# chanchanchan97/ICAFusion

Measured on NVIDIA H100. Metric: 640x512 RGB+IR pairs/sec end-to-end, higher is better.
Workload: dtype f16

## Files before the change

### icafusion_b200/_lib.py

```python
from __future__ import annotations

import ctypes as C
import os

_HERE = os.path.dirname(os.path.abspath(__file__))
LIB_PATH = os.path.join(_HERE, "libicaf_b200.so")

ACT_NONE, ACT_SILU, ACT_GELU = 0, 1, 2
EPI_BIAS_ROW, EPI_ADD_RES, EPI_SCALED_RES, EPI_LN_FOLD, EPI_EMIT_STATS = 1, 2, 4, 8, 16


class ConvGeom(C.Structure):
    _fields_ = [(n, C.c_int) for n in ("B", "Hi", "Wi", "Cin", "Ho", "Wo", "Cout", "kh", "kw", "stride", "pad",
                                       "k_pad", "w_rows", "act", "epi")]


class ConvIO(C.Structure):
    _fields_ = [("x", C.c_void_p), ("x_ld", C.c_int64), ("w", C.c_void_p), ("bias", C.c_void_p),
                ("res", C.c_void_p), ("res_ld", C.c_int64), ("y", C.c_void_p), ("y_ld", C.c_int64),
                ("alpha", C.c_void_p), ("beta", C.c_void_p),
                ("ln_stats", C.c_void_p), ("ln_colsum", C.c_void_p), ("ln_parts", C.c_int), ("ln_eps", C.c_float),
                ("stats_out", C.c_void_p)]


class ConvPlan(C.Structure):
    _fields_ = [(n, C.c_int) for n in ("kernel", "bn", "a_mode", "tile_w", "tile_h", "tiles_x", "tiles_y", "cblk", "halo",
                                       "stages", "splits", "grid_x", "grid_y", "grid_z", "cluster", "smem_bytes",
                                       "work_items", "ctas")]


class BottleneckIO(C.Structure):
    _fields_ = [("x", C.c_void_p), ("x_ld", C.c_int64), ("w1", C.c_void_p), ("b1", C.c_void_p), ("w3", C.c_void_p),
                ("b2", C.c_void_p), ("y", C.c_void_p), ("y_ld", C.c_int64)]


class LossHyp(C.Structure):
    _fields_ = [(n, C.c_float) for n in ("box", "obj", "cls", "cls_pw", "obj_pw", "anchor_t", "fl_gamma", "gr", "cp", "cn")] + \
               [("balance", C.c_float * 5)]


class AugTile(C.Structure):
    _fields_ = [("rgb", C.c_void_p), ("ir", C.c_void_p)] + \
               [(n, C.c_int) for n in ("H0", "W0", "h", "w", "x1a", "y1a", "x2a", "y2a", "x1b", "y1b", "xtab", "ytab")]


class AugSample(C.Structure):
    _fields_ = [("tile", AugTile * 4)] + [(n, C.c_int) for n in ("ntiles", "canvas", "warp", "flipud", "fliplr", "reserved")] + \
               [("lut", C.c_uint8 * (2 * 3 * 256))]


class ValSample(C.Structure):
    _fields_ = [("rgb", C.c_void_p), ("ir", C.c_void_p)] + \
               [(n, C.c_int) for n in ("H0", "W0", "h", "w", "top", "left", "mode", "xtab", "ytab", "sx", "sy", "reserved")]


KERNEL_TC = 0

_vp, _i, _i64, _f = C.c_void_p, C.c_int, C.c_int64, C.c_float
SIGNATURES = {
    "icaf_version": [],
    "icaf_last_error": [],
    "icaf_sm_count": [],
    "icaf_kernel_launches": [],
    "icaf_conv2d_fwd": [C.POINTER(ConvGeom), C.POINTER(ConvIO), _i, _vp],
    "icaf_conv2d_plan": [C.POINTER(ConvGeom), _i, _i, _i, C.POINTER(ConvPlan)],
    "icaf_conv2d_fwd_simt": [C.POINTER(ConvGeom), C.POINTER(ConvIO), _i, _vp],
    "icaf_bottleneck_fwd": [_i, _i, _i, C.POINTER(BottleneckIO), _i, _vp],
    "icaf_pack_image": [_vp, _i, _f, _i, _i, _i, _vp, _vp],
    "icaf_pack_image_s2d": [_vp, _i, _f, _i, _i, _i, _vp, _vp],
    "icaf_letterbox": [_vp, _i, _i, _i, _vp, _i, _i, _i, _i, _i, _i, _vp, _vp, _i, _vp],
    "icaf_sppf_pool": [_vp, _i64, _vp, _vp, _vp, _i64, _i, _i, _i, _i, _vp],
    "icaf_upsample2x": [_vp, _i64, _vp, _i64, _i, _i, _i, _i, _vp],
    "icaf_copy_channels": [_vp, _i64, _vp, _i64, _i64, _i, _vp],
    "icaf_prefetch_l2": [_vp, C.c_size_t, _vp],
    "icaf_dmff_pool_tokens": [_vp, _vp, _i64, _vp, _vp, _vp, _vp, _vp, _vp, _vp, _i, _i, _i, _i, _i, _i, _i, _vp],
    "icaf_row_stats": [_vp, _vp, _vp, _vp, _i64, _i, _vp],
    "icaf_layernorm": [_vp, _vp, _vp, _vp, _vp, _vp, _vp, _vp, _i64, _i, _f, _vp],
    "icaf_cross_attention": [_vp, _vp, _vp, _vp, _vp, _vp, _i, _i, _i, _i, _i, _vp],
    "icaf_cross_attention_simt": [_vp, _vp, _vp, _vp, _vp, _vp, _i, _i, _i, _i, _i, _vp],
    "icaf_dmff_upsample_cat": [_vp, _vp, _i, _vp, _vp, _i64, _vp, _i64, _i, _i, _i, _i, _i, _i, _i, _vp],
    "icaf_nms_workspace_bytes": [_i, _i],
    "icaf_nms": [_vp, _i, _i, _i, _f, _f, _i, C.c_uint64, _i, _vp, _vp, _vp, C.c_size_t, _vp],
    "icaf_nms_multi_label_workspace_bytes": [_i, _i, _i],
    "icaf_nms_multi_label": [_vp, _i, _i, _i, _f, _f, _i, C.c_uint64, _i, _vp, _vp, _vp, C.c_size_t, _vp],
    "icaf_match_detections_workspace_bytes": [_i],
    "icaf_match_detections": [_vp, _vp, _i, _i, _vp, _i, _vp, _i, _i, _vp, _i, _i, _vp, _vp, _vp, C.c_size_t, _vp],
    "icaf_kaist_mr_workspace_bytes": [_i, _i, _i],
    "icaf_kaist_mr": [_vp, _vp, _vp, _vp, _vp, _vp, _i, _i, _i, _vp, _vp, _i, _i, _vp, _vp, _vp, _vp, C.c_size_t, _vp],
    "icaf_kaist_round_detections": [_vp, _vp, _vp, _vp, _i, _i, _i, _vp, _vp, _vp],
    "icaf_loss_workspace_bytes": [_i, _i, _i, C.POINTER(C.c_int), C.POINTER(C.c_int), _i, _i],
    "icaf_compute_loss_fwd": [C.POINTER(C.c_void_p), _i, _i, C.POINTER(C.c_int), C.POINTER(C.c_int), _i, _i, _i, _i, _vp, _i,
                              C.POINTER(C.c_float), C.POINTER(LossHyp), _vp, _vp, C.c_size_t, _vp],
    "icaf_compute_loss_bwd": [C.POINTER(C.c_void_p), _i, _i, C.POINTER(C.c_int), C.POINTER(C.c_int), _i, _i, _i, _i, _vp, _i,
                              C.POINTER(C.c_float), C.POINTER(LossHyp), _vp, C.POINTER(C.c_void_p), _vp, C.c_size_t, _vp],
    "icaf_conv2d_wgrad_workspace_bytes": [C.POINTER(ConvGeom)],
    "icaf_conv2d_wgrad": [C.POINTER(ConvGeom), _vp, _i64, _vp, _i64, _vp, _f, _i, _vp, C.c_size_t, _vp],
    "icaf_zero_stuff2": [_vp, _vp, _i, _i, _i, _i, _i, _i, _vp],
    "icaf_colsum": [_vp, _i64, _i, _vp, _f, _i, _vp, C.c_size_t, _vp],
    "icaf_train_workspace_bytes": [_i],
    "icaf_bn_act_fwd": [_vp, _vp, _vp, _vp, _vp, _vp, _vp, _vp, _i64, _i, _f, _f, _i, _vp, C.c_size_t, _vp],
    "icaf_bn_act_bwd": [_vp, _vp, _vp, _vp, _vp, _vp, _vp, _vp, _vp, _i64, _i, _i, _f, _i, _vp, C.c_size_t, _vp],
    "icaf_bn_act_fwd_stats": [_vp, _i64, _i, _vp, _vp, C.c_size_t, _vp],
    "icaf_bn_act_fwd_apply": [_vp, _vp, _vp, _vp, _vp, _vp, _vp, _vp, _vp, _i64, _i, _f, _f, _i, _vp, C.c_size_t, _vp],
    "icaf_bn_act_bwd_sums": [_vp, _vp, _vp, _vp, _vp, _vp, _vp, _vp, _vp, _i64, _i, _i, _f, _i, _vp, C.c_size_t, _vp],
    "icaf_bn_act_bwd_apply": [_vp, _vp, _vp, _vp, _vp, _vp, _vp, _vp, _vp, _i64, _i, _i, _vp, C.c_size_t, _vp],
    "icaf_eltwise": [_i, _vp, _vp, _vp, _i64, _f, C.c_uint32, _vp],
    "icaf_layernorm_bwd": [_vp, _vp, _vp, _vp, _vp, _vp, _i64, _i, _f, _f, _i, _vp, C.c_size_t, _vp],
    "icaf_dot": [_vp, _vp, _i64, _i, _vp, _f, _i, _vp, C.c_size_t, _vp],
    "icaf_upsample2x_bwd": [_vp, _vp, _i, _i, _i, _i, _vp],
    "icaf_maxpool5_bwd": [_vp, _vp, _vp, _i, _i, _i, _i, _vp, C.c_size_t, _vp],
    "icaf_dmff_pool_tokens_bwd": [_vp, _vp, _i64, _vp, _vp, _vp, _vp, _vp, _i, _i, _i, _i, _i, _i, _i, _vp, C.c_size_t, _vp],
    "icaf_dmff_upsample_cat_bwd": [_vp, _i64, _vp, _vp, _i, _i, _i, _i, _i, _i, _i, _i, _vp],
    "icaf_pack_weight": [_vp, _i, _i, _i, _i, _i, _i, _i, _i, _vp, _vp],
    "icaf_pack_weight_pair": [_vp, _i, _i, _i, _i, _i, _i, _vp, _i, _i, _i, _vp, _vp],
    "icaf_set_seed_offset": [_vp],
    "icaf_cross_attention_train": [_vp, _vp, _vp, _vp, _i, _i, _i, _i, _i, _f, C.c_uint32, _vp],
    "icaf_cross_attention_bwd_workspace_bytes": [_i, _i, _i],
    "icaf_cross_attention_bwd": [_vp, _vp, _vp, _vp, _vp, _vp, _vp, _vp, _i, _i, _i, _i, _i, _f, C.c_uint32, _vp, C.c_size_t, _vp],
# ... 42 lines not shown
```

### icafusion_b200/csrc/conv_common.cuh

```cuda
#pragma once
#include "icaf_internal.cuh"

namespace icaf {

constexpr int BM = 128;
constexpr int BK = 64;
constexpr int kLag = 2;
constexpr int kThreads = 288;

enum AMode { A_GATHER = 0, A_TMA2D = 1, A_TMA4D = 2 };

struct ConvProblem {
  const __half* x; const float* bias; const __half* res; __half* y;
  const float* alpha; const float* beta;
  long long x_ld, res_ld, y_ld;
  const float2* ln_stats;
  const float* ln_s;
  float2* stats_out;
};
struct ConvParams {
  ConvProblem p[2];
  int M, N, K, k_pad;
  int B, Hi, Wi, Cin, Ho, Wo, kh, kw, stride, pad;
  int act, epi;
// ... 163 lines not shown
}

__device__ __forceinline__ void load_staged(uint32_t (&acc)[32], const float* p) {
#pragma unroll
  for (int q = 0; q < 8; ++q) {
    const float4 v = *reinterpret_cast<const float4*>(p + 4 * q);
    acc[4 * q] = __float_as_uint(v.x); acc[4 * q + 1] = __float_as_uint(v.y);
    acc[4 * q + 2] = __float_as_uint(v.z); acc[4 * q + 3] = __float_as_uint(v.w);
  }
}

template <bool XM>
__device__ __forceinline__ void epi_dispatch(int mode_act, const uint32_t (&acc)[32], const float* sb, float rbias, float alpha,
                                             float beta, const __half* rp, __half* yp, bool vec, int ncols, EpiRow& ex, int cb) {
  if (XM) {
    switch (mode_act) {
      case 9: epi_chunk<0, 0, 1>(acc, sb, rbias, alpha, beta, rp, yp, vec, ncols, ex, cb); break;
      case 10: epi_chunk<2, 0, 1>(acc, sb, rbias, alpha, beta, rp, yp, vec, ncols, ex, cb); break;
      default: epi_chunk<0, 2, 2>(acc, sb, rbias, alpha, beta, rp, yp, vec, ncols, ex, cb); break;
    }
  } else {
    switch (mode_act) {
      case 0: epi_chunk<0, 0>(acc, sb, rbias, alpha, beta, rp, yp, vec, ncols, ex, cb); break;
      case 1: epi_chunk<0, 1>(acc, sb, rbias, alpha, beta, rp, yp, vec, ncols, ex, cb); break;
      case 2: epi_chunk<0, 2>(acc, sb, rbias, alpha, beta, rp, yp, vec, ncols, ex, cb); break;
      case 3: epi_chunk<1, 0>(acc, sb, rbias, alpha, beta, rp, yp, vec, ncols, ex, cb); break;
      case 4: epi_chunk<1, 1>(acc, sb, rbias, alpha, beta, rp, yp, vec, ncols, ex, cb); break;
      case 5: epi_chunk<1, 2>(acc, sb, rbias, alpha, beta, rp, yp, vec, ncols, ex, cb); break;
      case 6: epi_chunk<2, 0>(acc, sb, rbias, alpha, beta, rp, yp, vec, ncols, ex, cb); break;
      case 7: epi_chunk<2, 1>(acc, sb, rbias, alpha, beta, rp, yp, vec, ncols, ex, cb); break;
      default: epi_chunk<2, 2>(acc, sb, rbias, alpha, beta, rp, yp, vec, ncols, ex, cb); break;
    }
  }
}

template <bool XM>
__device__ __forceinline__ int epi_mode_act(const ConvParams& P, bool has_res) {
  if (XM) return P.ln_parts > 0 ? (P.act == ICAF_ACT_GELU ? 10 : 9) : 11;
  return P.act * 3 + ((P.epi & ICAF_EPI_SCALED_RES) ? 2 : (has_res ? 1 : 0));
}

template <bool XM>
__device__ __forceinline__ void epi_staged_chunk(int mode_act, const uint32_t (&acc)[32], StagedRow& r, const float* sbias,
                                                 float alpha, float beta, int cb, int nb, int N) {
  const int ncols = min(32, N - nb);
  const bool vec = ncols == 32 && ((reinterpret_cast<uintptr_t>(r.yrow + nb) & 15) == 0) &&
                   (!r.rrow || (reinterpret_cast<uintptr_t>(r.rrow + nb) & 15) == 0);
  epi_dispatch<XM>(mode_act, acc, sbias + cb, r.rbias, alpha, beta, r.rrow ? r.rrow + nb : nullptr, r.yrow + nb, vec, ncols,
                   r.ex, cb);
}

constexpr int kOutHalfBytes = BM * 64 * 2;

template <int PP, int NA>
__device__ __forceinline__ void take_cols16(const float (&acc0)[NA], const float (&acc1)[NA], float (&v)[16]) {
  constexpr int Q = PP < NA / 8 ? PP : NA / 8 - 1;
#pragma unroll
  for (int e = 0; e < 8; ++e) { v[e] = acc0[8 * Q + e]; v[8 + e] = acc1[8 * Q + e]; }
}

template <int ACT, int RES>
__device__ __forceinline__ void epi_fragments(const float (&v)[16], uint32_t sa, const float* sb, const float (&rb)[4],
                                              float alpha, float beta) {
#pragma unroll
  for (int h = 0; h < 2; ++h) {
    uint32_t r[4];
    if (RES != 0) ldmatrix_x4(r, sa + 8192u * h);
#pragma unroll
    for (int k = 0; k < 4; ++k) {
      const float2 b = *reinterpret_cast<const float2*>(sb + 8 * (k >> 1));
      const float rbias = rb[2 * h + (k & 1)];
      float2 rf = make_float2(0.f, 0.f);
      if (RES != 0) rf = __half22float2(*reinterpret_cast<const __half2*>(&r[k]));
      r[k] = pack_half2(epi_value<ACT, RES>(v[8 * h + 2 * k], b.x, rbias, rf.x, alpha, beta),
                        epi_value<ACT, RES>(v[8 * h + 2 * k + 1], b.y, rbias, rf.y, alpha, beta));
    }
    stmatrix_x4(sa + 8192u * h, r);
  }
}

__device__ __forceinline__ void epi_fragments_dispatch(int mode_act, const float (&v)[16], uint32_t sa, const float* sb,
                                                       const float (&rb)[4], float alpha, float beta) {
  switch (mode_act) {
    case 0: epi_fragments<0, 0>(v, sa, sb, rb, alpha, beta); break;
    case 1: epi_fragments<0, 1>(v, sa, sb, rb, alpha, beta); break;
    case 2: epi_fragments<0, 2>(v, sa, sb, rb, alpha, beta); break;
    case 3: epi_fragments<1, 0>(v, sa, sb, rb, alpha, beta); break;
    case 4: epi_fragments<1, 1>(v, sa, sb, rb, alpha, beta); break;
    case 5: epi_fragments<1, 2>(v, sa, sb, rb, alpha, beta); break;
    case 6: epi_fragments<2, 0>(v, sa, sb, rb, alpha, beta); break;
    case 7: epi_fragments<2, 1>(v, sa, sb, rb, alpha, beta); break;
    default: epi_fragments<2, 2>(v, sa, sb, rb, alpha, beta); break;
  }
}

template <int NA>
__device__ __forceinline__ void epi_tile_fragments(int mode_act, const float (&acc0)[NA], const float (&acc1)[NA], uint32_t sout,
                                                   const float* sbias, const float (&rb)[4], float alpha, float beta, int w, int l) {
  const uint32_t sa = sout + uint32_t(16 * w + (l & 7) + 8 * ((l >> 3) & 1)) * 128u;
  const float* sb = sbias + 2 * (l & 3);
#pragma unroll 1
  for (int p = 0; p < NA / 8; ++p) {
    float v[16];
    switch (p) {
      case 0: take_cols16<0>(acc0, acc1, v); break;
      case 1: take_cols16<1>(acc0, acc1, v); break;
      case 2: take_cols16<2>(acc0, acc1, v); break;
      case 3: take_cols16<3>(acc0, acc1, v); break;
      case 4: take_cols16<4>(acc0, acc1, v); break;
      case 5: take_cols16<5>(acc0, acc1, v); break;
      case 6: take_cols16<6>(acc0, acc1, v); break;
      default: take_cols16<7>(acc0, acc1, v); break;
    }
    const uint32_t a = sa + uint32_t(p >> 2) * uint32_t(kOutHalfBytes) + (uint32_t((2 * (p & 3) + (l >> 4)) ^ (l & 7)) << 4);
    epi_fragments_dispatch(mode_act, v, a, sb + 16 * p, rb, alpha, beta);
  }
}

__device__ __forceinline__ void fragment_row_bias(float (&rb)[4], const ConvParams& P, const ConvProblem& pr, const TileOrigin& o,
                                                  int w, int l) {
  if ((P.epi & ICAF_EPI_BIAS_ROW) && pr.bias) {
#pragma unroll
    for (int q = 0; q < 4; ++q) {
      int mq;
      bool vq;
      tile_row(P, o, 16 * w + (l >> 2) + 8 * (q & 1) + 64 * (q >> 1), mq, vq);
      rb[q] = vq ? __ldg(pr.bias + mq) : 0.f;
    }
  }
}

template <int BN>
__device__ __forceinline__ void tma_store_tile(const ConvParams& P, const CUtensorMap* map, uint32_t s, int n0, const TileOrigin& o) {
  const int halves = (BN == 128 && n0 + 64 < P.N) ? 2 : 1;
  for (int hh = 0; hh < halves; ++hh) {
    const uint32_t src = s + uint32_t(hh * kOutHalfBytes);
    if (P.a_mode == A_TMA4D) tma_store_4d(map, src, n0 + 64 * hh, o.ox0, o.oy0, o.tb);
    else tma_store_2d(map, src, n0 + 64 * hh, o.m0);
  }
  bulk_commit_group();
}

template <int BN>
__device__ __forceinline__ void tma_load_tile(const ConvParams& P, const CUtensorMap* map, uint32_t s, uint32_t bar, int n0,
                                              const TileOrigin& o) {
  const int halves = (BN == 128 && n0 + 64 < P.N) ? 2 : 1;
  const uint32_t half_bytes = P.a_mode == A_TMA4D ? uint32_t(P.tw * P.th) * 128u : uint32_t(kOutHalfBytes);
  mbar_arrive_expect_tx(bar, uint32_t(halves) * half_bytes);
  for (int hh = 0; hh < halves; ++hh) {
    const uint32_t dst = s + uint32_t(hh * kOutHalfBytes);
    if (P.a_mode == A_TMA4D) tma_load_4d(dst, map, bar, n0 + 64 * hh, o.ox0, o.oy0, o.tb);
    else tma_load_2d(dst, map, bar, n0 + 64 * hh, o.m0);
  }
}

struct ConvPlan {
  int kernel;
  int bn;
  unsigned grid_x, grid_y, grid_z, cluster;
  int smem;
  int tiles, m_tiles, n_tiles;
  int sms;
  bool persist;
  bool stem;
  bool xm;
  int ctas;
};

}
```

### icafusion_b200/csrc/conv_gemm.cu

```cuda
#include <cstdlib>
#include <cstring>

#include "conv_common.cuh"

namespace icaf {

constexpr int kMaxStages = 10;
template <int BN>
struct SmemLayout {
  static constexpr int kABytes = BM * BK * 2;
  static constexpr int kBBytes = BN * BK * 2;
  static constexpr int kStageBytes = kABytes + kBBytes;
  static constexpr int kPitch = BN + 4;
  static constexpr int kAccBytes = BM * kPitch * 4;
  static constexpr int kTailBytes = 256 + BN * 4 + 1024;
  __host__ __device__ static int region(int stages) { return stages * kStageBytes > kAccBytes ? stages * kStageBytes : kAccBytes; }
  static int total(int stages) { return region(stages) + kTailBytes; }
};


template <int BN, bool kTmaA>
__device__ __forceinline__ void load_stage(const ConvParams& P, int a_mode, uint32_t sa, uint32_t bar, uint32_t bytes,
                                           const CUtensorMap* mw, const CUtensorMap* ma, int kb, int n0, const TileOrigin& o) {
  mbar_arrive_expect_tx(bar, bytes);
// ... 479 lines not shown
    auto hand_back = [&](int s) { if (l == 0) mbar_arrive(empty_bar(s)); };
    auto halo_back = [&](int h) { if (l == 0) mbar_arrive(halo_empty(h)); };
    const int g0 = j * nkb;
    if (j > 0) mbar_wait_quiet(order_bar(c), uint32_t((j >> 1) - (1 - c)) & 1u);
    int s_last, h_last = 0;
    if (halo) {
      halo_mma_loop(acc0, acc1, P, smem_base, kStages, g0, j * ncb, lane_px, l, full_bar, halo_full, hand_back, halo_back,
                    s_last, h_last);
    } else {
      s_last = mma_loop<128>(acc0, acc1, smem_base, kStages, nkb, g0 % kStages, uint32_t(g0 / kStages) & 1u, full_bar,
                             hand_back);
    }
    if (l == 0) mbar_arrive(order_bar(c ^ 1));
    wgmma_wait<0>();
    hand_back(s_last);
    if (halo) halo_back(h_last);

    if constexpr (!XM) {
      if (has_res) mbar_wait_quiet(res_bar(c), uint32_t(j >> 1) & 1u);
      epi_tile_fragments<64>(epi_mode_act<false>(P, has_res), acc0, acc1, sout, sbias, rb, alpha, beta, w, l);
      fence_proxy_async_smem();
      named_bar_sync(bar_id, 128);
      if (t == 0) {
        tma_store_tile<128>(P, pt.z ? &maps.y[1] : &maps.y[0], sout, n0, o);
        if (tile + 2 * int(gridDim.x) >= P.tiles) bulk_wait_group<0>();
      }
      continue;
    }

    const int mode_act = epi_mode_act<XM>(P, has_res);
    const float* arow = sacc + size_t(t) * PL::kPitch;
#pragma unroll 1
    for (int cc = 0; cc < 4; ++cc) {
      named_bar_sync(bar_id, 128);
      if (cc == 0) sbias[t] = bias_r;
      switch (cc) {
        case 0: stage_chunk<0>(acc0, acc1, sacc, w, l); break;
        case 1: stage_chunk<1>(acc0, acc1, sacc, w, l); break;
        case 2: stage_chunk<2>(acc0, acc1, sacc, w, l); break;
        default: stage_chunk<3>(acc0, acc1, sacc, w, l); break;
      }
      named_bar_sync(bar_id, 128);
      const int cb = 32 * cc;
      if (sr.mvalid && n0 + cb < P.N) {
        uint32_t acc[32];
        load_staged(acc, arow);
        epi_staged_chunk<XM>(mode_act, acc, sr, sbias, alpha, beta, cb, n0 + cb, P.N);
      }
    }
    if (mode_act == 11 && sr.mvalid && n0 < P.N) epi_row_emit(sr.ex, P, pr, sr.m, n0, min(n0 + 128, P.N));
  }
}

constexpr int kStemThreads = 128;
struct StemLayout {
  static constexpr int kFilterBytes = 3 * SmemLayout<64>::kBBytes;
  static constexpr int kBiasOff = kFilterBytes;
  static constexpr int kBarOff = kBiasOff + 64 * 4;
  static constexpr int kHaloOff = kFilterBytes + 1024;
  __host__ __device__ static int pitch(int Wo) { return (Wo < BM ? Wo : BM) + 2; }
  __host__ __device__ static int runs(int Wo) { return 1 + (BM - 1 + Wo - 1) / Wo; }
  static int total(int Wo) {
    const int halo = runs(Wo) * 3 * pitch(Wo) * 32;
    return kHaloOff + (halo > kOutHalfBytes ? halo : kOutHalfBytes) + 1024;
  }
};

__global__ void __launch_bounds__(kStemThreads, 4)
conv_stem_kernel(const ConvParams P, const __grid_constant__ ConvMaps maps) {
  extern __shared__ uint8_t smem_raw[];
  using SL = StemLayout;
  const uint32_t smem_base = (smem_u32(smem_raw) + 1023u) & ~1023u;
  uint8_t* smem_gen = smem_raw + (smem_base - smem_u32(smem_raw));
  const uint32_t bar = smem_base + SL::kBarOff;
  const uint32_t halo = smem_base + SL::kHaloOff;
  float* sbias = reinterpret_cast<float*>(smem_gen + SL::kBiasOff);

  pdl_launch_dependents();
  const int t = threadIdx.x, w = t >> 5, l = t & 31;
  const int bz = blockIdx.z, n0 = blockIdx.y * 64;
  const ConvProblem pr = pick_problem(P, bz);
  const TileOrigin o{int(blockIdx.x) * BM, 0, 0, 0};
  const int g0 = o.m0 / P.Wo, ox0 = o.m0 - g0 * P.Wo;
  const int len0 = min(P.Wo - ox0, BM);
  const int nruns = 1 + (BM - len0 + P.Wo - 1) / P.Wo;
  const int pitch = SL::pitch(P.Wo);
  int lane_hp[2];
#pragma unroll
  for (int hm = 0; hm < 2; ++hm) {
    const int r = 64 * hm + 16 * w + (l & 7) + 8 * ((l >> 3) & 1);
    int j = 0, p = r;
    if (r >= len0) {
      const int q = (r - len0) / P.Wo;
      j = 1 + q;
      p = r - len0 - q * P.Wo;
    }
    lane_hp[hm] = 3 * j * pitch + p;
  }
  if (t == 0) {
    mbar_init(bar, 1);
    fence_mbar_init();
  }
  if (t == 32) {
    tma_prefetch_desc(bz ? &maps.w[1] : &maps.w[0]);
    tma_prefetch_desc(bz ? &maps.y[1] : &maps.y[0]);
  }
// ... 184 lines not shown
  constexpr int kSmemCap = 227 * 1024;
  const int mt = P.a_mode == A_TMA4D ? P.B * P.tiles_x * P.tiles_y : (P.M + BM - 1) / BM;
  if (P.a_mode == A_TMA4D && !(P.tw >= 1 && P.th >= 1 && P.tw * P.th <= BM && P.tiles_x * P.tw >= P.Wo && P.tiles_y * P.th >= P.Ho &&
                               P.cblk == 64 && P.Cin % 64 == 0))
    return set_error(ICAF_ERR_BAD_ARG, "conv2d(tc): 4-D tiles must cover the map with at most 128 pixels each, 64-channel blocks");
  unsigned gx = unsigned(mt), gy = unsigned((P.N + BN - 1) / BN), gz = unsigned(n_io);
  const long long tiles = (long long)gx * gy * gz;
  const int budget = (tiles <= pl.sms || BN > 64) ? kSmemCap : (kSmemCap / 2 - 1024);
  int stages = (budget - L::kTailBytes) / L::kStageBytes;
  const int nkb = P.k_pad / BK;
  if (stages > nkb) stages = nkb;
  if (stages > kMaxStages) stages = kMaxStages;
  if (stages < 2) stages = 2;
  int splits = 1;
  if (tiles * 2 <= pl.sms && nkb >= 8) {
    splits = int(pl.sms / tiles);
    if (splits > 8) splits = 8;
    if (splits > nkb / 4) splits = nkb / 4;
    if (splits < 1) splits = 1;
  }
  if (splits > 1) {
    const int per = (nkb + splits - 1) / splits;
    if (stages > per) stages = per < 2 ? 2 : per;
    gx *= splits;
  }
  if (stages > kMaxStages || L::total(stages) > kSmemCap)
    return set_error(ICAF_ERR_BAD_ARG, "conv2d(tc): shared-memory plan exceeds the ring / 227 KB");
  P.stages = stages;
  P.splits = splits;
  pl.kernel = ICAF_KERNEL_TC; pl.bn = BN;
  pl.grid_x = gx; pl.grid_y = gy; pl.grid_z = gz; pl.cluster = unsigned(splits);
  pl.smem = L::total(stages);
  pl.tiles = int(tiles); pl.m_tiles = mt; pl.n_tiles = int(gy);
  pl.persist = false; pl.ctas = int(gx * gy * gz);
  return ICAF_OK;
}

static int plan_persist(ConvParams& P, ConvPlan& pl) {
  constexpr int kSmemCap = 227 * 1024;
  const bool halo = !pl.xm && P.a_mode == A_TMA4D && P.kh == 3 && P.kw == 3 && P.stride == 1 && P.pad == 1;
  P.halo_bytes = halo ? ((P.tw + 2) * (P.th + 2) * 128 + 1023) / 1024 * 1024 : 0;
  int stages = kMaxStages;
  while (stages > 2 && PersistLayout::total(stages, P.halo_bytes) > kSmemCap) --stages;
  if (PersistLayout::total(stages, P.halo_bytes) > kSmemCap)
    return set_error(ICAF_ERR_BAD_ARG, "conv2d(persist): shared-memory plan exceeds 227 KB");
  P.stages = stages;
  P.m_tiles = pl.m_tiles; P.n_tiles = pl.n_tiles; P.tiles = pl.tiles;
  pl.persist = true;
  pl.ctas = pl.tiles < pl.sms ? pl.tiles : pl.sms;
  pl.smem = PersistLayout::total(stages, P.halo_bytes);
  return ICAF_OK;
}

template <int BN>
static int encode_maps(const ConvParams& P, const __half* const (&w)[2], const icaf_conv_geom* g, int n_io, bool out_maps,
                       ConvMaps& maps) {
  memset(&maps, 0, sizeof(maps));
  for (int i = 0; i < n_io; ++i) {
    int rc = encode_tmap_2d(&maps.w[i], w[i], (uint64_t)P.k_pad, (uint64_t)g->w_rows, (uint64_t)P.k_pad * 2, BK, BN);
    if (rc) return rc;
    const ConvProblem& pr = P.p[i];
    if (P.a_mode == A_TMA2D)
      rc = encode_tmap_2d(&maps.a[i], pr.x, (uint64_t)P.Cin, (uint64_t)P.M, (uint64_t)pr.x_ld * 2, BK, BM);
    else if (P.a_mode == A_TMA4D && P.halo_bytes)
      rc = encode_tmap_nhwc(&maps.a[i], pr.x, P.Cin, P.Wi, P.Hi, P.B, pr.x_ld, BK, P.tw + 2, P.th + 2, 1, 1);
    else if (P.a_mode == A_TMA4D)
      rc = encode_tmap_nhwc(&maps.a[i], pr.x, P.Cin, P.Wi, P.Hi, P.B, pr.x_ld, BK, P.tw * P.stride, P.th * P.stride, P.stride,
                            P.stride);
    if (rc) return rc;
    if (out_maps) {
      auto out_map = [&](CUtensorMap* m, const __half* base, long long ld) {
        return P.a_mode != A_TMA4D ? encode_tmap_2d(m, base, (uint64_t)P.N, (uint64_t)P.M, (uint64_t)ld * 2, 64, BM)
                                   : encode_tmap_nhwc(m, base, P.N, P.Wo, P.Ho, P.B, ld, 64, P.tw, P.th, 1, 1);
      };
      if ((rc = out_map(&maps.y[i], pr.y, pr.y_ld))) return rc;
      if (pr.res && (rc = out_map(&maps.res[i], pr.res, pr.res_ld))) return rc;
    }
  }
  if (n_io == 1) { maps.w[1] = maps.w[0]; maps.a[1] = maps.a[0]; maps.y[1] = maps.y[0]; maps.res[1] = maps.res[0]; }
  return ICAF_OK;
}

template <int BN>
static int launch_conv(const ConvParams& P, const ConvPlan& pl, const __half* const (&w)[2], const icaf_conv_geom* g, int n_io,
                       cudaStream_t st) {
  void (*kernel)(ConvParams, ConvMaps) = pl.xm ? conv_gemm_tc_kernel<BN, true> : conv_gemm_tc_kernel<BN, false>;
  if (pl.persist) kernel = pl.xm ? conv_gemm_persist_kernel<true> : conv_gemm_persist_kernel<false>;
  if (pl.stem) kernel = conv_stem_kernel;
  static bool configured[3][2][kMaxDevices] = {};
  const int family = pl.stem ? 2 : (pl.persist ? 1 : 0);
  if (int rc = configure_smem(kernel, 227 * 1024, configured[family][pl.xm], "conv2d: cudaFuncSetAttribute")) return rc;
  ConvMaps maps;
  if (int rc = encode_maps<BN>(P, w, g, n_io, P.tma_epi != 0, maps)) return rc;
  const dim3 grid = pl.persist ? dim3(unsigned(pl.ctas)) : dim3(pl.grid_x, pl.grid_y, pl.grid_z);
  const int threads = pl.persist ? kPersistThreads : (pl.stem ? kStemThreads : kThreads);
  return launch_kc("conv2d_fwd", kernel, grid, dim3(threads), (size_t)pl.smem, st, pl.cluster, P, maps);
}

static int plan_conv(const icaf_conv_geom* g, int n_io, int sms, bool tma_out, ConvParams& P, ConvPlan& pl) {
  memset(&pl, 0, sizeof(pl));
  pl.sms = sms;
  if (sms < 1) return set_error(ICAF_ERR_BAD_ARG, "conv2d: SM count must be positive");
  pl.xm = (P.epi & (ICAF_EPI_LN_FOLD | ICAF_EPI_EMIT_STATS)) != 0;
  plan_a_mode(g, P);
  const long long mt = P.a_mode == A_TMA4D ? (long long)P.B * P.tiles_x * P.tiles_y : (P.M + BM - 1) / BM;
  auto ctas = [&](int bn) { return mt * ((P.N + bn - 1) / bn) * n_io; };
  int bn = 32;
  if (P.N > 64 && ctas(128) >= sms) bn = 128;
  else if (P.N > 32 && ctas(64) >= sms) bn = 64;
  int rc;
  switch (bn) {
    case 128:
      rc = plan_tc<128>(P, n_io, pl);
      if (!rc && (pl.xm || tma_out) && P.a_mode != A_GATHER && P.splits == 1 && pl.tiles > sms) rc = plan_persist(P, pl);
      break;
    case 64:
      rc = plan_tc<64>(P, n_io, pl);
      if (!rc && !pl.xm && tma_out && P.a_mode == A_GATHER && P.splits == 1 && P.Cin == 16 && P.kh == 3 && P.kw == 3 &&
          P.stride == 1 && P.pad == 1 && !(P.epi & (ICAF_EPI_ADD_RES | ICAF_EPI_SCALED_RES))) {
        P.stages = 1;
        pl.stem = true;
        pl.smem = StemLayout::total(P.Wo);
      }
      break;
    default: rc = plan_tc<32>(P, n_io, pl); break;
  }
  if (rc) return rc;
  P.tma_epi = !pl.xm && (pl.persist || (tma_out && P.splits == 1 && pl.bn >= 64)) ? 1 : 0;
  return ICAF_OK;
}

}

using namespace icaf;


extern "C" int icaf_conv2d_plan(const icaf_conv_geom* g, int n_io, int sm_count, int pair_mode, icaf_conv_plan* out) {
  if (!out) return set_error(ICAF_ERR_BAD_ARG, "conv2d_plan: null output");
  ConvParams P;
  int rc = fill_geom(g, n_io, P);
  if (rc) return rc;
  ConvPlan pl;
  (void)pair_mode;
  rc = plan_conv(g, n_io, sm_count, true, P, pl);
  if (rc) return rc;
  out->kernel = pl.kernel; out->bn = pl.bn; out->a_mode = P.a_mode;
  out->tile_w = P.tw; out->tile_h = P.th; out->tiles_x = P.tiles_x; out->tiles_y = P.tiles_y;
  out->cblk = P.cblk; out->halo = 0; out->stages = P.stages; out->splits = P.splits;
  out->grid_x = int(pl.grid_x); out->grid_y = int(pl.grid_y); out->grid_z = int(pl.grid_z); out->cluster = int(pl.cluster);
  out->smem_bytes = pl.smem; out->work_items = pl.tiles; out->ctas = pl.ctas;
  return ICAF_OK;
}

extern "C" int icaf_conv2d_fwd(const icaf_conv_geom* g, const icaf_conv_io* io, int n_io, void* stream) {
  ConvParams P;
  const __half* w[2];
  int rc = fill_params(g, io, n_io, P, w);
  if (rc) return rc;
  bool tma_out = true;
  for (int i = 0; i < n_io; ++i) {
    const ConvProblem& pr = P.p[i];
    tma_out = tma_out && (reinterpret_cast<uintptr_t>(pr.y) & 15) == 0 && pr.y_ld % 8 == 0 &&
              (!pr.res || ((reinterpret_cast<uintptr_t>(pr.res) & 15) == 0 && pr.res_ld % 8 == 0));
  }
  ConvPlan pl;
  rc = plan_conv(g, n_io, sm_count_cached(), tma_out, P, pl);
  if (rc) return rc;
  cudaStream_t st = (cudaStream_t)stream;
  switch (pl.bn) {
    case 128: return launch_conv<128>(P, pl, w, g, n_io, st);
    case 64: return launch_conv<64>(P, pl, w, g, n_io, st);
    case 32: return launch_conv<32>(P, pl, w, g, n_io, st);
    default: return set_error(ICAF_ERR_BAD_ARG, "conv2d: the planner produced an unknown tile width");
  }
}

extern "C" int icaf_conv2d_fwd_simt(const icaf_conv_geom* g, const icaf_conv_io* io, int n_io, void* stream) {
  SimtParams S;
  int rc = fill_params(g, io, n_io, S.P, S.w);
  if (rc) return rc;
  long long total = (long long)S.P.M * S.P.N;
  dim3 grid(blocks_for(total, 256), 1, n_io);
  return launch_k("conv2d_fwd_simt", conv_gemm_simt_kernel, dim3(grid), dim3(256), 0, (cudaStream_t)stream, S);
}
```

### include/icaf_b200.h

```cpp
#ifndef ICAF_B200_H
#define ICAF_B200_H

#include <stddef.h>
#include <stdint.h>

#ifdef __cplusplus
extern "C" {
#endif

#define ICAF_OK 0
#define ICAF_ERR_BAD_ARG 1
#define ICAF_ERR_UNSUPPORTED 2
#define ICAF_ERR_CUDA 3

#define ICAF_ACT_NONE 0
#define ICAF_ACT_SILU 1
#define ICAF_ACT_GELU 2

#define ICAF_EPI_BIAS_ROW 1
#define ICAF_EPI_ADD_RES 2
#define ICAF_EPI_SCALED_RES 4
#define ICAF_EPI_LN_FOLD 8
#define ICAF_EPI_EMIT_STATS 16

int icaf_version(void);
const char* icaf_last_error(void);
long long icaf_kernel_launches(void);
int icaf_sm_count(void);

typedef struct {
  int B, Hi, Wi, Cin;
  int Ho, Wo, Cout;
  int kh, kw, stride, pad;
  int k_pad;
  int w_rows;
  int act;
  int epi;
} icaf_conv_geom;

typedef struct {
  const void* x;     int64_t x_ld;
  const void* w;
  const float* bias;
  const void* res;   int64_t res_ld;
  void* y;           int64_t y_ld;
  const float* alpha;
  const float* beta;
  const float* ln_stats;
  const float* ln_colsum;
  int ln_parts;
  float ln_eps;
  float* stats_out;
} icaf_conv_io;

int icaf_conv2d_fwd(const icaf_conv_geom* g, const icaf_conv_io* io, int n_io, void* stream);

#define ICAF_KERNEL_TC 0
typedef struct {
  int kernel;
  int bn;
  int a_mode;
  int tile_w, tile_h, tiles_x, tiles_y;
  int cblk;
  int halo;
  int stages, splits;
  int grid_x, grid_y, grid_z, cluster;
  int smem_bytes;
  int work_items;
  int ctas;
} icaf_conv_plan;
int icaf_conv2d_plan(const icaf_conv_geom* g, int n_io, int sm_count, int pair_mode, icaf_conv_plan* out);

int icaf_conv2d_fwd_simt(const icaf_conv_geom* g, const icaf_conv_io* io, int n_io, void* stream);

typedef struct {
  const void* x;     int64_t x_ld;
  const void* w1;    const float* b1;
  const void* w3;    const float* b2;
  void* y;           int64_t y_ld;
} icaf_bottleneck_io;
int icaf_bottleneck_fwd(int B, int H, int W, const icaf_bottleneck_io* io, int n_io, void* stream);

int icaf_pack_image(const void* src, int src_dtype, float scale, int B, int H, int W, void* dst, void* stream);

int icaf_letterbox(const void* src, int B, int H0, int W0, void* dst, int H, int W, int top, int left, int new_h, int new_w,
                   const int* xtab, const int* ytab, int pad_value, void* stream);

#define ICAF_VAL_COPY 0
#define ICAF_VAL_LINEAR 1
#define ICAF_VAL_AREA_FAST 2
#define ICAF_VAL_AREA 3
typedef struct {
  const void* rgb; const void* ir;
  int H0, W0;
  int h, w;
  int top, left;
  int mode;
  int xtab, ytab;
  int sx, sy;
  int reserved;
} icaf_val_sample;

size_t icaf_val_stage_params_bytes(int B, int n_words);

int icaf_val_stage(const void* params, size_t params_bytes, int B, int H, int W, int n_words, void* out, void* stream);

int icaf_pack_image_s2d(const void* src, int src_dtype, float scale, int B, int H, int W, void* dst, void* stream);

int icaf_sppf_pool(const void* x, int64_t x_ld, void* y1, void* y2, void* y3, int64_t y_ld, int B, int H, int W,
                   int C, void* stream);

int icaf_upsample2x(const void* x, int64_t x_ld, void* y, int64_t y_ld, int B, int H, int W, int C, void* stream);

int icaf_prefetch_l2(const void* ptr, size_t bytes, void* stream);

int icaf_copy_channels(const void* x, int64_t x_ld, void* y, int64_t y_ld, int64_t pixels, int C, void* stream);

int icaf_dmff_pool_tokens(const void* x_vis, const void* x_ir, int64_t x_ld, const void* pos_vis, const void* pos_ir,
                          const float* mix, void* tok_vis, void* tok_ir, float* stats_vis, float* stats_ir, int B, int H,
                          int W, int C, int nh, int nw, int n_pad, void* stream);

int icaf_layernorm(const void* x0, const void* x1, const float* g0, const float* b0, const float* g1,
                   const float* b1, void* y0, void* y1, int64_t rows, int C, float eps, void* stream);

// ... 136 lines not shown
```

Before: 2206.

## Add warp-specialized streaming 1x1 conv kernel for memory-bound small-K GEMMs

Adds a persistent conv1x1 kernel with one TMA producer warpgroup and two ping-pong consumer pairs of warpgroups. Each pair computes 64-row halves of a 128-row tile, so one pair's epilogue and TMA store overlap the other pair's MMA. The planner routes memory-bound 1x1 convs (TMA2D, K<=256, bytes moved outweigh FLOPs by a fixed ratio) to it. The aim is to hide load and store latency on bandwidth-limited layers. The cost is extra barrier ordering complexity and register rebalancing. A per-device runtime switch can disable it.

New measurement: 2207, median of 6. Within noise of the previous version (+0.0%).

```diff
diff --git a/icafusion_b200/_lib.py b/icafusion_b200/_lib.py
--- a/icafusion_b200/_lib.py
+++ b/icafusion_b200/_lib.py
@@ -26,7 +26,7 @@
 class ConvPlan(C.Structure):
     _fields_ = [(n, C.c_int) for n in ("kernel", "bn", "a_mode", "tile_w", "tile_h", "tiles_x", "tiles_y", "cblk", "halo",
                                        "stages", "splits", "grid_x", "grid_y", "grid_z", "cluster", "smem_bytes",
-                                       "work_items", "ctas")]
+                                       "work_items", "ctas", "kind")]
 
 
 class BottleneckIO(C.Structure):
@@ -55,6 +55,7 @@
 
 
 KERNEL_TC = 0
+CONV_ONE_TILE, CONV_PERSIST, CONV_STEM, CONV_STREAM = 0, 1, 2, 3
 
 _vp, _i, _i64, _f = C.c_void_p, C.c_int, C.c_int64, C.c_float
 SIGNATURES = {
@@ -64,6 +65,7 @@
     "icaf_kernel_launches": [],
     "icaf_conv2d_fwd": [C.POINTER(ConvGeom), C.POINTER(ConvIO), _i, _vp],
     "icaf_conv2d_plan": [C.POINTER(ConvGeom), _i, _i, _i, C.POINTER(ConvPlan)],
+    "icaf_conv1x1_stream_enable": [_i, _i],
     "icaf_conv2d_fwd_simt": [C.POINTER(ConvGeom), C.POINTER(ConvIO), _i, _vp],
     "icaf_bottleneck_fwd": [_i, _i, _i, C.POINTER(BottleneckIO), _i, _vp],
     "icaf_pack_image": [_vp, _i, _f, _i, _i, _i, _vp, _vp],
diff --git a/icafusion_b200/csrc/conv_common.cuh b/icafusion_b200/csrc/conv_common.cuh
--- a/icafusion_b200/csrc/conv_common.cuh
+++ b/icafusion_b200/csrc/conv_common.cuh
@@ -239,18 +239,18 @@
 
 constexpr int kOutHalfBytes = BM * 64 * 2;
 
-template <int PP, int NA>
+template <int PP, int NA, int NH = 2>
 __device__ __forceinline__ void take_cols16(const float (&acc0)[NA], const float (&acc1)[NA], float (&v)[16]) {
   constexpr int Q = PP < NA / 8 ? PP : NA / 8 - 1;
 #pragma unroll
-  for (int e = 0; e < 8; ++e) { v[e] = acc0[8 * Q + e]; v[8 + e] = acc1[8 * Q + e]; }
-}
-
-template <int ACT, int RES>
+  for (int e = 0; e < 8; ++e) { v[e] = acc0[8 * Q + e]; if (NH == 2) v[8 + e] = acc1[8 * Q + e]; }
+}
+
+template <int ACT, int RES, int NH = 2>
 __device__ __forceinline__ void epi_fragments(const float (&v)[16], uint32_t sa, const float* sb, const float (&rb)[4],
                                               float alpha, float beta) {
 #pragma unroll
-  for (int h = 0; h < 2; ++h) {
+  for (int h = 0; h < NH; ++h) {
     uint32_t r[4];
     if (RES != 0) ldmatrix_x4(r, sa + 8192u * h);
 #pragma unroll
@@ -266,22 +266,23 @@
   }
 }
 
+template <int NH = 2>
 __device__ __forceinline__ void epi_fragments_dispatch(int mode_act, const float (&v)[16], uint32_t sa, const float* sb,
                                                        const float (&rb)[4], float alpha, float beta) {
   switch (mode_act) {
-    case 0: epi_fragments<0, 0>(v, sa, sb, rb, alpha, beta); break;
-    case 1: epi_fragments<0, 1>(v, sa, sb, rb, alpha, beta); break;
-    case 2: epi_fragments<0, 2>(v, sa, sb, rb, alpha, beta); break;
-    case 3: epi_fragments<1, 0>(v, sa, sb, rb, alpha, beta); break;
-    case 4: epi_fragments<1, 1>(v, sa, sb, rb, alpha, beta); break;
-    case 5: epi_fragments<1, 2>(v, sa, sb, rb, alpha, beta); break;
-    case 6: epi_fragments<2, 0>(v, sa, sb, rb, alpha, beta); break;
-    case 7: epi_fragments<2, 1>(v, sa, sb, rb, alpha, beta); break;
-    default: epi_fragments<2, 2>(v, sa, sb, rb, alpha, beta); break;
-  }
-}
-
-template <int NA>
+    case 0: epi_fragments<0, 0, NH>(v, sa, sb, rb, alpha, beta); break;
+    case 1: epi_fragments<0, 1, NH>(v, sa, sb, rb, alpha, beta); break;
+    case 2: epi_fragments<0, 2, NH>(v, sa, sb, rb, alpha, beta); break;
+    case 3: epi_fragments<1, 0, NH>(v, sa, sb, rb, alpha, beta); break;
+    case 4: epi_fragments<1, 1, NH>(v, sa, sb, rb, alpha, beta); break;
+    case 5: epi_fragments<1, 2, NH>(v, sa, sb, rb, alpha, beta); break;
+    case 6: epi_fragments<2, 0, NH>(v, sa, sb, rb, alpha, beta); break;
+    case 7: epi_fragments<2, 1, NH>(v, sa, sb, rb, alpha, beta); break;
+    default: epi_fragments<2, 2, NH>(v, sa, sb, rb, alpha, beta); break;
+  }
+}
+
+template <int NA, int NH = 2>
 __device__ __forceinline__ void epi_tile_fragments(int mode_act, const float (&acc0)[NA], const float (&acc1)[NA], uint32_t sout,
                                                    const float* sbias, const float (&rb)[4], float alpha, float beta, int w, int l) {
   const uint32_t sa = sout + uint32_t(16 * w + (l & 7) + 8 * ((l >> 3) & 1)) * 128u;
@@ -290,17 +291,17 @@
   for (int p = 0; p < NA / 8; ++p) {
     float v[16];
     switch (p) {
-      case 0: take_cols16<0>(acc0, acc1, v); break;
-      case 1: take_cols16<1>(acc0, acc1, v); break;
-      case 2: take_cols16<2>(acc0, acc1, v); break;
-      case 3: take_cols16<3>(acc0, acc1, v); break;
-      case 4: take_cols16<4>(acc0, acc1, v); break;
-      case 5: take_cols16<5>(acc0, acc1, v); break;
-      case 6: take_cols16<6>(acc0, acc1, v); break;
-      default: take_cols16<7>(acc0, acc1, v); break;
+      case 0: take_cols16<0, NA, NH>(acc0, acc1, v); break;
+      case 1: take_cols16<1, NA, NH>(acc0, acc1, v); break;
+      case 2: take_cols16<2, NA, NH>(acc0, acc1, v); break;
+      case 3: take_cols16<3, NA, NH>(acc0, acc1, v); break;
+      case 4: take_cols16<4, NA, NH>(acc0, acc1, v); break;
+      case 5: take_cols16<5, NA, NH>(acc0, acc1, v); break;
+      case 6: take_cols16<6, NA, NH>(acc0, acc1, v); break;
+      default: take_cols16<7, NA, NH>(acc0, acc1, v); break;
     }
     const uint32_t a = sa + uint32_t(p >> 2) * uint32_t(kOutHalfBytes) + (uint32_t((2 * (p & 3) + (l >> 4)) ^ (l & 7)) << 4);
-    epi_fragments_dispatch(mode_act, v, a, sb + 16 * p, rb, alpha, beta);
+    epi_fragments_dispatch<NH>(mode_act, v, a, sb + 16 * p, rb, alpha, beta);
   }
 }
 
@@ -350,6 +351,7 @@
   int sms;
   bool persist;
   bool stem;
+  bool stream;
   bool xm;
   int ctas;
 };
diff --git a/icafusion_b200/csrc/conv_gemm.cu b/icafusion_b200/csrc/conv_gemm.cu
--- a/icafusion_b200/csrc/conv_gemm.cu
+++ b/icafusion_b200/csrc/conv_gemm.cu
@@ -555,6 +555,152 @@
   }
 }
 
+constexpr int kStreamThreads = 5 * 128;
+constexpr int kStreamRegsProducer = 24, kStreamRegsConsumer = 112;
+static_assert(128 * kStreamRegsProducer + 4 * 128 * kStreamRegsConsumer <= kStreamThreads * 96, "register split exceeds the launch's");
+struct StreamLayout {
+  static constexpr int kOutBytes = 2 * kOutHalfBytes;
+  __host__ __device__ static int bar_off(int stages) { return stages * SmemLayout<128>::kStageBytes + 2 * kOutBytes; }
+  static int total(int stages) { return bar_off(stages) + 256 + 2 * 128 * 4 + 1024; }
+};
+
+template <class FullBar, class HandBack>
+__device__ __forceinline__ int mma_loop_rows64(float (&acc)[64], uint32_t a_off, uint32_t smem_base, int kStages, int nkb, int s0,
+                                               uint32_t ph0, FullBar full_bar, HandBack hand_back) {
+  int s = s0, s_prev = s0;
+  uint32_t ph = ph0;
+  for (int kb = 0; kb < nkb; ++kb) {
+    mbar_wait_quiet(full_bar(s), ph);
+    const uint32_t sa = smem_base + s * SmemLayout<128>::kStageBytes;
+    wgmma_fence();
+#pragma unroll
+    for (int k = 0; k < BK / 16; ++k)
+      wgmma_ss<0, 0>(acc, gmma_desc_sw128(sa + a_off + 32 * k), gmma_desc_sw128(sa + SmemLayout<128>::kABytes + 32 * k),
+                     (kb | k) != 0);
+    wgmma_commit();
+    wgmma_wait<1>();
+    if (kb > 0) hand_back(s_prev);
+    s_prev = s;
+    if (++s == kStages) { s = 0; ph ^= 1; }
+  }
+  return s_prev;
+}
+
+__global__ void __launch_bounds__(kStreamThreads, 1)
+conv1x1_stream_kernel(const ConvParams P, const __grid_constant__ ConvMaps maps) {
+  extern __shared__ uint8_t smem_raw[];
+  const uint32_t smem_base = (smem_u32(smem_raw) + 1023u) & ~1023u;
+  using L = SmemLayout<128>;
+  using SL = StreamLayout;
+  const int kStages = P.stages;
+  const uint32_t ring_bytes = uint32_t(kStages * L::kStageBytes);
+  const uint32_t bar_off = uint32_t(SL::bar_off(kStages));
+  const uint32_t bar_base = smem_base + bar_off;
+  auto full_bar = [&](int s) { return bar_base + 8u * s; };
+  auto empty_bar = [&](int s) { return bar_base + 8u * (kMaxStages + s); };
+  auto order_bar = [&](int p) { return bar_base + 8u * (2 * kMaxStages + p); };
+  auto res_bar = [&](int p) { return bar_base + 8u * (2 * kMaxStages + 2 + p); };
+  static_assert(8 * (2 * kMaxStages + 4) <= 256, "barriers");
+  uint8_t* smem_gen = smem_raw + (smem_base - smem_u32(smem_raw));
+
+  pdl_launch_dependents();
+  const int tid = threadIdx.x;
+  const int wg = tid >> 7;
+  const int nkb = P.k_pad / BK;
+  const bool has_res = (P.epi & (ICAF_EPI_ADD_RES | ICAF_EPI_SCALED_RES)) != 0;
+  if (tid == 0) {
+    for (int s = 0; s < kStages; ++s) {
+      mbar_init(full_bar(s), 1);
+      mbar_init(empty_bar(s), 8);
+    }
+    for (int p = 0; p < 2; ++p) {
+      mbar_init(order_bar(p), 8);
+      mbar_init(res_bar(p), 1);
+    }
+    fence_mbar_init();
+  }
+  if (tid == 32) {
+    tma_prefetch_desc(&maps.w[0]);
+    tma_prefetch_desc(&maps.a[0]);
+    if (P.tiles > P.m_tiles * P.n_tiles) { tma_prefetch_desc(&maps.w[1]); tma_prefetch_desc(&maps.a[1]); }
+    tma_prefetch_desc(&maps.y[0]);
+    if (has_res) tma_prefetch_desc(&maps.res[0]);
+  }
+  __syncthreads();
+  pdl_wait();
+
+  if (wg == 4) {
+    setmaxnreg_dec<kStreamRegsProducer>();
+    if (tid < 4 * 128 + 32 && elect_one()) {
+      int s = 0;
+      uint32_t ph = 0;
+      for (int tile = blockIdx.x; tile < P.tiles; tile += gridDim.x) {
+        const PersistTile pt = persist_tile(P, tile);
+        const CUtensorMap* mw = pt.z ? &maps.w[1] : &maps.w[0];
+        const CUtensorMap* ma = pt.z ? &maps.a[1] : &maps.a[0];
+        for (int kb = 0; kb < nkb; ++kb) {
+          mbar_wait_quiet(empty_bar(s), ph ^ 1);
+          load_stage<128, true>(P, A_TMA2D, smem_base + s * L::kStageBytes, full_bar(s), L::kStageBytes, mw, ma, kb, pt.n0, pt.o);
+          if (++s == kStages) { s = 0; ph ^= 1; }
+        }
+      }
+    }
+    return;
+  }
+
+  setmaxnreg_inc<kStreamRegsConsumer>();
+  const int p = wg >> 1, h = wg & 1;
+  const int t = tid & 127, w = t >> 5, l = t & 31;
+  const int bar_id = 1 + p;
+  const uint32_t sout = smem_base + ring_bytes + uint32_t(p * SL::kOutBytes);
+  float* sbias = reinterpret_cast<float*>(smem_gen + bar_off + 256 + p * 128 * 4);
+  const int mode_act = epi_mode_act<false>(P, has_res);
+  const bool storer = h == 0 && t == 0;
+  for (int tile = blockIdx.x + p * gridDim.x; tile < P.tiles; tile += 2 * gridDim.x) {
+    const int j = (tile - int(blockIdx.x)) / int(gridDim.x);
+    const PersistTile pt = persist_tile(P, tile);
+    const ConvProblem pr = pick_problem(P, pt.z);
+    const int n0 = pt.n0;
+    float alpha = 0.f, beta = 1.f;
+    if (P.epi & ICAF_EPI_SCALED_RES) { alpha = __ldg(pr.alpha); beta = __ldg(pr.beta); }
+    float rb[4] = {0.f, 0.f, 0.f, 0.f};
+    const TileOrigin oh{pt.o.m0 + 64 * h, 0, 0, 0};
+    fragment_row_bias(rb, P, pr, oh, w, l);
+    if (has_res && storer) {
+      bulk_wait_group_read<0>();
+      tma_load_tile<128>(P, pt.z ? &maps.res[1] : &maps.res[0], sout, res_bar(p), n0, pt.o);
+    }
+    if (h == 0) sbias[t] = (pr.bias && !(P.epi & ICAF_EPI_BIAS_ROW) && n0 + t < P.N) ? __ldg(pr.bias + n0 + t) : 0.f;
+    named_bar_sync(bar_id, 256);
+
+    float acc[64];
+#pragma unroll
+    for (int i = 0; i < 64; ++i) acc[i] = 0.f;
+    auto hand_back = [&](int s) { if (l == 0) mbar_arrive(empty_bar(s)); };
+    const int g0 = j * nkb;
+    if (j > 0) mbar_wait_quiet(order_bar(p), uint32_t((j >> 1) - (1 - p)) & 1u);
+    const int s_last = mma_loop_rows64(acc, uint32_t(h * 64 * 128), smem_base, kStages, nkb, g0 % kStages,
+                                       uint32_t(g0 / kStages) & 1u, full_bar, hand_back);
+    if (l == 0) mbar_arrive(order_bar(p ^ 1));
+    wgmma_wait<0>();
+    hand_back(s_last);
+
+    if (has_res) {
+      mbar_wait_quiet(res_bar(p), uint32_t(j >> 1) & 1u);
+    } else {
+      if (storer) bulk_wait_group_read<0>();
+      named_bar_sync(bar_id, 256);
+    }
+    epi_tile_fragments<64, 1>(mode_act, acc, acc, sout + uint32_t(h * 64 * 128), sbias, rb, alpha, beta, w, l);
+    fence_proxy_async_smem();
+    named_bar_sync(bar_id, 256);
+    if (storer) {
+      tma_store_tile<128>(P, pt.z ? &maps.y[1] : &maps.y[0], sout, n0, pt.o);
+      if (tile + 2 * int(gridDim.x) >= P.tiles) bulk_wait_group<0>();
+    }
+  }
+}
+
 constexpr int kStemThreads = 128;
 struct StemLayout {
   static constexpr int kFilterBytes = 3 * SmemLayout<64>::kBBytes;
@@ -845,6 +991,23 @@
   return ICAF_OK;
 }
 
+static bool moves_more_than_multiplies(const ConvParams& P) {
+  const unsigned __int128 M = unsigned(P.M), N = unsigned(P.N), K = unsigned(P.K);
+  const unsigned res = (P.epi & (ICAF_EPI_ADD_RES | ICAF_EPI_SCALED_RES)) ? 2u : 1u;
+  return 98900u * (M * K + res * M * N + N * K) >= 335u * M * N * K;
+}
+
+static void plan_stream(ConvParams& P, ConvPlan& pl) {
+  constexpr int kSmemCap = 227 * 1024;
+  int stages = kMaxStages;
+  while (stages > 2 && StreamLayout::total(stages) > kSmemCap) --stages;
+  P.stages = stages;
+  pl.stream = true;
+  pl.smem = StreamLayout::total(stages);
+}
+
+static bool g_stream_off[kMaxDevices] = {};
+
 template <int BN>
 static int encode_maps(const ConvParams& P, const __half* const (&w)[2], const icaf_conv_geom* g, int n_io, bool out_maps,
                        ConvMaps& maps) {
@@ -880,17 +1043,18 @@
   void (*kernel)(ConvParams, ConvMaps) = pl.xm ? conv_gemm_tc_kernel<BN, true> : conv_gemm_tc_kernel<BN, false>;
   if (pl.persist) kernel = pl.xm ? conv_gemm_persist_kernel<true> : conv_gemm_persist_kernel<false>;
   if (pl.stem) kernel = conv_stem_kernel;
-  static bool configured[3][2][kMaxDevices] = {};
-  const int family = pl.stem ? 2 : (pl.persist ? 1 : 0);
+  if (pl.stream) kernel = conv1x1_stream_kernel;
+  static bool configured[4][2][kMaxDevices] = {};
+  const int family = pl.stream ? 3 : (pl.stem ? 2 : (pl.persist ? 1 : 0));
   if (int rc = configure_smem(kernel, 227 * 1024, configured[family][pl.xm], "conv2d: cudaFuncSetAttribute")) return rc;
   ConvMaps maps;
   if (int rc = encode_maps<BN>(P, w, g, n_io, P.tma_epi != 0, maps)) return rc;
   const dim3 grid = pl.persist ? dim3(unsigned(pl.ctas)) : dim3(pl.grid_x, pl.grid_y, pl.grid_z);
-  const int threads = pl.persist ? kPersistThreads : (pl.stem ? kStemThreads : kThreads);
+  const int threads = pl.stream ? kStreamThreads : (pl.persist ? kPersistThreads : (pl.stem ? kStemThreads : kThreads));
   return launch_kc("conv2d_fwd", kernel, grid, dim3(threads), (size_t)pl.smem, st, pl.cluster, P, maps);
 }
 
-static int plan_conv(const icaf_conv_geom* g, int n_io, int sms, bool tma_out, ConvParams& P, ConvPlan& pl) {
+static int plan_conv(const icaf_conv_geom* g, int n_io, int sms, bool tma_out, bool stream, ConvParams& P, ConvPlan& pl) {
   memset(&pl, 0, sizeof(pl));
   pl.sms = sms;
   if (sms < 1) return set_error(ICAF_ERR_BAD_ARG, "conv2d: SM count must be positive");
@@ -906,6 +1070,8 @@
     case 128:
       rc = plan_tc<128>(P, n_io, pl);
       if (!rc && (pl.xm || tma_out) && P.a_mode != A_GATHER && P.splits == 1 && pl.tiles > sms) rc = plan_persist(P, pl);
+      if (!rc && pl.persist && stream && !pl.xm && P.a_mode == A_TMA2D && P.K <= 256 && moves_more_than_multiplies(P))
+        plan_stream(P, pl);
       break;
     case 64:
       rc = plan_tc<64>(P, n_io, pl);
@@ -935,9 +1101,10 @@
   if (rc) return rc;
   ConvPlan pl;
   (void)pair_mode;
-  rc = plan_conv(g, n_io, sm_count, true, P, pl);
+  rc = plan_conv(g, n_io, sm_count, true, true, P, pl);
   if (rc) return rc;
-  out->kernel = pl.kernel; out->bn = pl.bn; out->a_mode = P.a_mode;
+  out->kernel = pl.kernel;
+  out->kind = pl.stream ? ICAF_CONV_STREAM : (pl.stem ? ICAF_CONV_STEM : (pl.persist ? ICAF_CONV_PERSIST : ICAF_CONV_ONE_TILE)); out->bn = pl.bn; out->a_mode = P.a_mode;
   out->tile_w = P.tw; out->tile_h = P.th; out->tiles_x = P.tiles_x; out->tiles_y = P.tiles_y;
   out->cblk = P.cblk; out->halo = 0; out->stages = P.stages; out->splits = P.splits;
   out->grid_x = int(pl.grid_x); out->grid_y = int(pl.grid_y); out->grid_z = int(pl.grid_z); out->cluster = int(pl.cluster);
@@ -956,8 +1123,10 @@
     tma_out = tma_out && (reinterpret_cast<uintptr_t>(pr.y) & 15) == 0 && pr.y_ld % 8 == 0 &&
               (!pr.res || ((reinterpret_cast<uintptr_t>(pr.res) & 15) == 0 && pr.res_ld % 8 == 0));
   }
+  const int dev = current_device();
+  const bool stream_on = !(dev >= 0 && dev < kMaxDevices && g_stream_off[dev]);
   ConvPlan pl;
-  rc = plan_conv(g, n_io, sm_count_cached(), tma_out, P, pl);
+  rc = plan_conv(g, n_io, sm_count_cached(), tma_out, stream_on, P, pl);
   if (rc) return rc;
   cudaStream_t st = (cudaStream_t)stream;
   switch (pl.bn) {
@@ -968,6 +1137,12 @@
   }
 }
 
+extern "C" int icaf_conv1x1_stream_enable(int device, int enable) {
+  if (device < 0 || device >= kMaxDevices) return set_error(ICAF_ERR_BAD_ARG, "conv1x1_stream_enable: device ordinal out of range");
+  g_stream_off[device] = enable == 0;
+  return ICAF_OK;
+}
+
 extern "C" int icaf_conv2d_fwd_simt(const icaf_conv_geom* g, const icaf_conv_io* io, int n_io, void* stream) {
   SimtParams S;
   int rc = fill_params(g, io, n_io, S.P, S.w);
diff --git a/include/icaf_b200.h b/include/icaf_b200.h
--- a/include/icaf_b200.h
+++ b/include/icaf_b200.h
@@ -68,8 +68,15 @@
   int smem_bytes;
   int work_items;
   int ctas;
+  int kind;
 } icaf_conv_plan;
+#define ICAF_CONV_ONE_TILE 0
+#define ICAF_CONV_PERSIST 1
+#define ICAF_CONV_STEM 2
+#define ICAF_CONV_STREAM 3
 int icaf_conv2d_plan(const icaf_conv_geom* g, int n_io, int sm_count, int pair_mode, icaf_conv_plan* out);
+
+int icaf_conv1x1_stream_enable(int device, int enable);
 
 int icaf_conv2d_fwd_simt(const icaf_conv_geom* g, const icaf_conv_io* io, int n_io, void* stream);
 
```
